# eric612/Mobilenet-YOLO-Pytorch

Hardware: AMD Instinct MI355X
Metric: images/sec MobileNetV2-YOLO 352x352 fwd+bwd @ bs256 (higher is better)
Workload: dtype f32; 1 GPU; MobileNetV2-YOLO 352x352 bs=256/GPU fwd+loss+bwd fp32 (BASELINE configs[1]); global_batch=256, parallelism=dp1

## Files before the change

### include/mnyolo.h

```cpp
#ifndef MNYOLO_H
#define MNYOLO_H

#include <stddef.h>
#include <stdint.h>

#ifdef __cplusplus
extern "C" {
#endif
#pragma GCC visibility push(default)

#define MNY_OK 0
#define MNY_EINVAL (-1)
#define MNY_EHIP (-2)
#define MNY_EUNSUPPORTED (-3)

#define MNY_ACT_NONE 0
#define MNY_ACT_RELU6 1
#define MNY_ACT_LEAKY 2
#define MNY_ACT_RELU 3
#define MNY_ACT_HSWISH 4
#define MNY_ACT_HSIGMOID 5

int mny_version(void);
const char* mny_last_error(void);
// ... 469 lines not shown
                     const float* w_exp, const float* e_scale, const float* e_shift, const float* e_mean, const float* e_invstd,
                     const float* e_gamma, const float* w_dw, const float* addend, float* dx, float* dw_exp, float* dgamma_e, float* dbeta_e,
                     float* dw_dw, float* dw_ws, float* ws, float* in_red, int N, int H, int W, int K, int C, int stride, void* stream);

int mny_stemdw_supported(int N, int H, int W, int Cout, int s_act, int d_act);
int mny_stemdw_bwd_parts(int N, int H, int W, int Cout);
size_t mny_stemdw_bwd_ws_floats(int N, int H, int W, int Cout);
int mny_stemdw_bwd(const float* gd, const float* d, const float* d_scale, const float* d_shift, int d_act, const float* d_coef,
                   const float* s, const float* s_scale, const float* s_shift, const float* s_mean, const float* s_invstd,
                   const float* s_gamma, int s_act, const float* x_nchw, const float* w_stem, const float* w_dw,
                   float* dw_stem, float* dgamma_s, float* dbeta_s, float* dw_dw, float* dw_ws, float* ws,
                   int N, int H, int W, int Cout, void* stream);

int mny_pj_bwd_supported(int64_t M, int Ki, int No, int d_act);
int mny_pj_bwd_parts(int64_t M, int Ki, int No);
int mny_pj_bwd(const float* g, const float* y, const float* coef, const float* d, const float* d_scale, const float* d_shift,
               const float* d_mean, const float* d_invstd, int d_act, const float* w, float* gd, float* dw, float* dw_ws, float* red,
               int64_t M, int Ki, int No, void* stream);
int mny_pj_bwd_supported_bf16(int64_t M, int Ki, int No, int d_act);
int mny_pj_bwd_parts_bf16(int64_t M, int Ki, int No);
int mny_pj_bwd_bf16(const void* g, const void* y, const float* coef, const void* d, const float* d_scale, const float* d_shift,
                    const float* d_mean, const float* d_invstd, int d_act, const float* w, void* gd, float* dw, float* dw_ws, float* red,
                    int64_t M, int Ki, int No, void* stream);

typedef struct mny_gate_cut_job {
    const float* w1;
    const float* w2;
    void* wq;
    int32_t C, R;
} mny_gate_cut_job;
int mny_gate_supported(int64_t M, int C, int R);
int mny_gate_parts(int64_t M);
int mny_gate_bwd_parts(int64_t M);
int mny_gate_bwd_red3_supported(int C, int R);
size_t mny_gate_wq_bytes(int C, int R);
int mny_gate_cut_batch_bf16(const mny_gate_cut_job* jobs, int njobs, void* stream);
int mny_gate_stats1_bf16(const void* y3, const float* s3, const float* b3, const void* wq, float* stats, int64_t M, int C, int R,
                         void* stream);
int mny_gate_stats2_bf16(const void* y3, const float* s3, const float* b3, const void* wq, const float* sc1, const float* sh1,
                         float* stats, int64_t M, int C, int R, void* stream);
int mny_gate_fwd_bf16(const void* y3, const float* s3, const float* b3, const void* wq, const float* sc1, const float* sh1,
                      const float* sc2, const float* sh2, const void* add_x, const float* add_scale, const float* add_shift,
                      int add_act, void* out, int64_t M, int C, int R, void* stream);
int mny_gate_bwd1_bf16(const void* y3, const float* s3, const float* b3, const void* dout, const void* wq, const float* sc1,
                       const float* sh1, const float* sc2, const float* sh2, const float* mean2, const float* invstd2, float* red2,
                       int64_t M, int C, int R, void* stream);
// ... 23 lines not shown
```

### mobilenet-yolo-pytorch_amd/_lib.py

```python
import ctypes
import os
from ctypes import c_char_p, c_double, c_float, c_int, c_int32, c_int64, c_size_t, c_void_p

from . import switches

HERE = os.path.dirname(os.path.abspath(__file__))
LIB_PATH = switches.get("MNY_LIB") or os.path.join(HERE, "libmnyolo.so")

ACT_NONE, ACT_RELU6, ACT_LEAKY, ACT_RELU, ACT_HSWISH, ACT_HSIGMOID = 0, 1, 2, 3, 4, 5
ROUTE_TILE_V1, ROUTE_DMA_F32, ROUTE_DMA_X6, ROUTE_THIN, ROUTE_WIDE, ROUTE_WGRAD_STREAM, ROUTE_WAVE16 = 0, 1, 2, 3, 4, 5, 6


class MnyError(RuntimeError):
    pass


class YoloHead(ctypes.Structure):
    _fields_ = [("N", c_int), ("g", c_int), ("A", c_int), ("C", c_int), ("n_anchors_all", c_int),
                ("ignore_thresh", c_float), ("iou_thresh", c_float), ("iou_weighting", c_float)]


P = c_void_p
_SIGS = {
    "mny_version": (c_int, []),
# ... 13 lines not shown
    "mny_dw_wgrad_parts": (c_int, [c_int] * 6),
    "mny_dw_bnbwd_supported": (c_int, [c_int, c_int]),
    "mny_dw_bnbwd_parts": (c_int, [c_int] * 4),
    "mny_dw_bnbwd_parts_k": (c_int, [c_int] * 6),
    "mny_dw_bnbwd": (c_int, [P, P, P, P, c_int, P, P, P, P, c_int, P, P, P, P, P, c_int, c_int, c_int, c_int, c_int, c_int, P]),
    "mny_dw_bnbwd_s2_parts": (c_int, [c_int] * 4),
    "mny_dw_bnbwd_s2": (c_int, [P, P, P, P, c_int, P, P, P, P, c_int, P, P, P, P, P, c_int, c_int, c_int, c_int, P]),
    "mny_dw_bnbwd_red": (c_int, [P, P, P, P, c_int, P, P, P, P, c_int, P, P, P, P, P, P, P, P, c_int, c_int, c_int, c_int, c_int, c_int, P]),
    "mny_exdw_supported": (c_int, [c_int] * 6),
    "mny_exdw_stat_parts": (c_int, [c_int64, c_int, c_int]),
    "mny_exdw_stats": (c_int, [P, P, P, c_int, P, P, c_int64, c_int, c_int, P]),
    "mny_exdw_fwd_parts": (c_int, [c_int] * 6),
    "mny_exdw_fwd": (c_int, [P, P, P, c_int, P, P, P, P, P, P, c_int, c_int, c_int, c_int, c_int, c_int, P]),
    "mny_exdw_bwd_parts": (c_int, [c_int] * 6),
    "mny_exdw_bwd_ws_floats": (c_size_t, [c_int] * 6),
    "mny_exdw_bwd": (c_int, [P, P, P, P, c_int, P, P, P, P, c_int, P, P, P, P, P, P, P, P, P, P, P, P, P, P, P,
                             c_int, c_int, c_int, c_int, c_int, c_int, P]),
    "mny_exdw_bwd_red_parts": (c_int, [c_int] * 6),
    "mny_exdw_bwd_red": (c_int, [P, P, P, P, c_int, P, P, P, P, c_int, P, P, P, P, P, P, P, P, P, P, P, P, P, P, P, P, P, P,
                                 c_int, c_int, c_int, c_int, c_int, c_int, P]),
    "mny_pj_bwd_supported": (c_int, [c_int64, c_int, c_int, c_int]),
    "mny_pj_bwd_parts": (c_int, [c_int64, c_int, c_int]),
    "mny_pj_bwd": (c_int, [P, P, P, P, P, P, P, P, c_int, P, P, P, P, P, c_int64, c_int, c_int, P]),
    "mny_stemdw_supported": (c_int, [c_int] * 6),
    "mny_stemdw_bwd_parts": (c_int, [c_int] * 4),
    "mny_stemdw_bwd_ws_floats": (c_size_t, [c_int] * 4),
    "mny_stemdw_bwd": (c_int, [P, P, P, P, c_int, P, P, P, P, P, P, P, c_int, P, P, P, P, P, P, P, P, P, c_int, c_int, c_int, c_int, P]),
    "mny_adamw_step": (c_int, [P, c_int, c_double, c_double, c_double, c_double, c_double, c_int64, P]),
    "mny_sgd_step": (c_int, [P, c_int, c_double, c_double, c_double, c_double, c_int, c_int, P]),
    "mny_ema_update": (c_int, [P, c_int, c_double, P]),
    "mny_swap_chunks": (c_int, [P, c_int, P]),
    "mny_grad_clip_parts": (c_int, [c_int64]),
    "mny_grad_clip": (c_int, [P, c_int, c_int, c_double, P, P, P]),
    "mny_pw_fwd": (c_int, [P, P, P, c_int, P, P, P, P, P, c_int64, c_int, c_int, P]),
    "mny_pw_stat_parts": (c_int, [c_int64, c_int, c_int]),
    "mny_pw_wgrad": (c_int, [P, P, P, c_int, P, P, P, P, c_int64, c_int, c_int, P]),
    "mny_pw_wgrad_ws_floats": (c_size_t, [c_int64, c_int, c_int]),
    "mny_pw_bnbwd_supported": (c_int, [c_int64, c_int, c_int]),
    "mny_pw_bnbwd_ws_floats": (c_size_t, [c_int64, c_int, c_int]),
    "mny_pw_bnbwd": (c_int, [P, P, P, P, c_int, P, P, P, P, P, P, c_int, P, P, P, P, P, P, P, c_int64, c_int, c_int, P]),
    "mny_pw_dgrad_bnred_supported": (c_int, [c_int64, c_int, c_int, c_int]),
    "mny_pw_dgrad_bnred_parts": (c_int, [c_int64, c_int, c_int]),
    "mny_pw_dgrad_bnred": (c_int, [P, P, P, P, P, P, c_int, P, P, P, c_int64, c_int, c_int, P]),
    "mny_pw_dgrad_bnred_add_supported": (c_int, [c_int64, c_int, c_int, c_int]),
    "mny_pw_dgrad_bnred_add": (c_int, [P, P, P, P, P, P, P, c_int, P, P, P, c_int64, c_int, c_int, P]),
    "mny_pw_route": (c_int, [c_int, c_int, c_int64, c_int, c_int]),
# ... 139 lines not shown
```

### mobilenet-yolo-pytorch_amd/csrc/common.h

```cpp
#pragma once
#include <hip/hip_runtime.h>
#include <stdint.h>
#include <stdio.h>
#include <stdlib.h>
#include <type_traits>

#include "../../include/mnyolo.h"

namespace mny {

void set_error(const char* fmt, ...);
int check_launch(const char* what);
bool allow_lds(const void* kernel, size_t bytes);

#define MNY_REQUIRE(cond, ...)                 \
    do {                                       \
        if (!(cond)) {                         \
            mny::set_error(__VA_ARGS__);       \
            return MNY_EINVAL;                 \
        }                                      \
    } while (0)

constexpr int kWave = 64;
constexpr int kMaxParts = 1024;
// ... 116 lines not shown
    if constexpr (B < E) {
        f(std::integral_constant<int, B>{});
        static_for<B + 1, E>(f);
    }
}
#define MNY_LGKM_WAIT(first) asm volatile("s_waitcnt lgkmcnt(0)" : "+v"(first))
#define MNY_LGKM_DEP(x) asm volatile("" : "+v"(x))

template <int N>
__device__ __forceinline__ void wait_vmcnt() { asm volatile("s_waitcnt vmcnt(%0)" ::"n"(N) : "memory"); }

#define MNY_SWITCHES(X)                                                                                                              \
    X(GEMM_V1, "MNY_GEMM_V1", kFlag, 0, 1, "pointwise forward / data gradients on the first-generation tile kernels")                \
    X(WGRAD_V1, "MNY_WGRAD_V1", kFlag, 0, 1, "pointwise weight gradients on the first-generation tile kernel")                       \
    X(WGRAD_NO_XCD, "MNY_WGRAD_NO_XCD", kFlag, 0, 1, "weight-gradient workgroups in plain order, not grouped per XCD")               \
    X(X6, "MNY_X6", kInt, -1, 1, "six-product bf16 GEMM: 0 = never (fp32 MFMA), 1 = wherever supported, -1 = per-shape rule")        \
    X(NO_W6, "MNY_NO_W6", kFlag, 0, 1, "no pre-cut weight operand for the six-product GEMM")                                         \
    X(NO_WIDE, "MNY_NO_WIDE", kFlag, 0, 1, "no barrier-free short-reduction kernel (pwwide.hip)")                                    \
    X(NO_WGS, "MNY_NO_WGS", kFlag, 0, 1, "no stream weight-gradient kernel (pwwgs.hip)")                                             \
    X(NO_THIN, "MNY_NO_THIN", kFlag, 0, 1, "no vector-ALU kernel for K = 8..32 (pwthin.hip)")                                        \
    X(NO_PWT, "MNY_NO_PWT", kFlag, 0, 1, "no wave-per-16-pixels thin pointwise kernel (gate.hip)")                                   \
    X(NO_PWE, "MNY_NO_PWE", kFlag, 0, 1, "no wave form of the thin expand unit backward (gate.hip)")                                 \
    X(NO_PJBWD, "MNY_NO_PJBWD", kFlag, 0, 1, "no fused projection backward (pjbwd.hip, gate.hip)")                                   \
    X(NO_LR, "MNY_NO_LR", kFlag, 0, 1, "no low-rank BatchNorm backward of the wide expand units (lrbwd.hip)")                        \
    X(NO_EXDW, "MNY_NO_EXDW", kFlag, 0, 1, "no fused expand + depthwise unit: the materialised path")                                \
    X(EXDW_STATS, "MNY_EXDW_STATS", kWord, 0, 0, "gram (default) | direct: how mny_exdw_stats forms its sums")                       \
    X(NO_STEMDW, "MNY_NO_STEMDW", kFlag, 0, 1, "no fused stem + depthwise backward (stemdw.hip)")                                    \
    X(STEM_WGRAD_VALU, "MNY_STEM_WGRAD_VALU", kFlag, 0, 1, "stem weight gradient on the vector ALU, not the matrix cores")           \
    X(DW_V1, "MNY_DW_V1", kFlag, 0, 1, "3x3 depthwise forward on the first-generation sliding-window kernel")                        \
    X(NO_DWT5, "MNY_NO_DWT5", kFlag, 0, 1, "no tile form of the 5x5 depthwise unit backward")                                        \
    X(DWT3, "MNY_DWT3", kInt, -1, 1, "tile form of the 3x3 depthwise unit backward: 0 / 1, -1 = per-shape rule")                     \
    X(DWTF, "MNY_DWTF", kInt, -1, 1, "tile form of the depthwise forward: 0 / 1, -1 = per-shape rule")                               \
    X(NMS_SMALL, "MNY_NMS_SMALL", kFlag, 0, 0, "NMS buckets of any size through the one-workgroup path")
enum SwitchType { kFlag, kInt, kWord };
enum Switch {
#define X(id, name, type, def, latch, doc) SW_##id,
    MNY_SWITCHES(X)
#undef X
    SW_COUNT
};
int sw(Switch id);

struct CgLayout {
    int cg_total;
    int chunks;
    int cgb;
// ... 79 lines not shown
```

### mobilenet-yolo-pytorch_amd/csrc/pwwide.hip

```cpp
#include <mutex>
#include <vector>

#include "common.h"
#include "x6.h"

namespace mny {

struct WideArgs {
    const float* A; const float* in_scale; const float* in_shift; int in_act;
    const float* W;
    float* C; float* stats;
    int64_t M; int K, N;
    int gx, n_blocks; int64_t ntiles;
    const float* rY; const float* r_scale; const float* r_shift; const float* r_mean; const float* r_invstd; int r_act;
    const float* addend;
    const float* bias;
};

template <int KS, int TNB, int XF, int MODE>
__global__ __launch_bounds__(256) __attribute__((amdgpu_waves_per_eu(2, 2))) void pw_wide_kernel(WideArgs p) {
    constexpr int BN = 32 * TNB;
    constexpr bool TWO_ACC = false;
    extern __shared__ __attribute__((aligned(16))) float smem[];
    float* sB = smem;
    float* sScale = sB + TNB * KS * 3 * 256;
    float* sShift = sScale + KS * 16;
    const int tid = threadIdx.x, lane = tid & 63;
    const int wave = __builtin_amdgcn_readfirstlane(tid >> 6);
    const int lrow = lane & 31, khalf = lane >> 5;
    const int bid = blockIdx.x, xcd = bid & 7, local = bid >> 3;
    const int y = local % p.n_blocks, x = (local / p.n_blocks) * 8 + xcd;
    if (x >= p.gx) return;
    const int n0 = y * BN;
    const int K = p.K, N = p.N;

    for (int c = tid; c < TNB * KS * 64; c += 256) {
        const int sidx = c >> 6, l = c & 63, j = l & 31, h = l >> 5;
        const int u = sidx / KS, s = sidx - u * KS;
        const int n = n0 + u * 32 + j;
        const int k0 = s * 16 + 4 * h, k1 = k0 + 8;
        const float* src = p.W + (int64_t)(n < N ? n : 0) * K;
        const float4 v0 = (n < N && k0 < K) ? ld4(src + k0) : f4zero();
        const float4 v1 = (n < N && k1 < K) ? ld4(src + k1) : f4zero();
        bf16x8_t hh, mm, ll;
        x6_split(v4f_t{v0.x, v0.y, v0.z, v0.w}, v4f_t{v1.x, v1.y, v1.z, v1.w}, hh, mm, ll);
        float* dst = sB + (sidx * 3) * 256 + l * 4;
        *reinterpret_cast<v4f_t*>(dst) = __builtin_bit_cast(v4f_t, hh);
        *reinterpret_cast<v4f_t*>(dst + 256) = __builtin_bit_cast(v4f_t, mm);
        *reinterpret_cast<v4f_t*>(dst + 512) = __builtin_bit_cast(v4f_t, ll);
    }
    if ((XF != 0 && MODE < 2) || MODE == 4) {
        const bool has = p.in_scale != nullptr;
        for (int k = tid; k < KS * 16; k += 256) {
            sScale[k] = k < K ? (has ? p.in_scale[k] : 1.f) : 0.f;
            sShift[k] = (k < K && has) ? p.in_shift[k] : 0.f;
        }
    }
    __syncthreads();

    const float slope = act_slope(p.in_act), hi = act_hi(p.in_act);
    const int quad = lrow >> 2, jq = lane & 3;
    const float rslope = act_slope(p.r_act), rhi = act_hi(p.r_act);
    const bool rhsig = p.r_act == MNY_ACT_HSIGMOID;
    float s1[TNB], s2[TNB];
#pragma unroll
    for (int u = 0; u < TNB; ++u) { s1[u] = 0.f; s2[u] = 0.f; }

    const float* bl = sB + lane * 4;
    const float* scl = sScale + 4 * khalf;
    const float* shl = sShift + 4 * khalf;
    const int64_t nslots = (int64_t)p.gx * 4;
    const unsigned rowb = (unsigned)N * 4u;
    float4 g[2 * KS];
    float ry[MODE >= 2 ? 16 : 1], ra[MODE >= 3 ? 16 : 1];
    auto load_g = [&](int64_t tile, int s) {
        const int64_t r = tile * 32 + lrow;
        const float* row = p.A + (r < p.M ? r : p.M - 1) * K;
        int k0 = 16 * s + 4 * khalf, k1 = k0 + 8;
        if (s == KS - 1) { k0 = k0 < K ? k0 : 0; k1 = k1 < K ? k1 : 0; }
        g[2 * s] = ld4(row + k0); g[2 * s + 1] = ld4(row + k1);
    };
    auto load_r = [&](int64_t tile, int u) {
        const int col = n0 + u * 32 + lrow, cc = col < N ? col : 0;
        unsigned voff = (unsigned)(4 * khalf) * rowb + (unsigned)cc * 4u;
        asm volatile("" : "+v"(voff));
        const float* ub = p.rY + tile * 32 * N;
#pragma unroll
        for (int r = 0; r < 16; ++r) ry[r] = ld1(at_bytes(ub + (int64_t)(8 * (r >> 2) + (r & 3)) * N, voff));
        if constexpr (MODE >= 3) {
            const float* ua = p.addend + tile * 32 * N;
#pragma unroll
            for (int r = 0; r < 16; ++r) ra[r] = ld1(at_bytes(ua + (int64_t)(8 * (r >> 2) + (r & 3)) * N, voff));
        }
    };

    auto do_tile = [&](const int64_t tile, const int64_t next) {
        const int64_t wrow = tile * 32;
        bf16x8_t ah[KS], am[KS], al[KS];
#pragma unroll
        for (int s = 0; s < KS; ++s) {
            const float4 a0 = g[2 * s], a1 = g[2 * s + 1];
            float z[8] = {a0.x, a0.y, a0.z, a0.w, a1.x, a1.y, a1.z, a1.w};
            if ((XF != 0 && MODE < 2) || MODE == 4) {
                v4f_t c0 = *reinterpret_cast<const v4f_t*>(scl + 16 * s), c1 = *reinterpret_cast<const v4f_t*>(scl + 16 * s + 8);
                v4f_t h0 = *reinterpret_cast<const v4f_t*>(shl + 16 * s), h1 = *reinterpret_cast<const v4f_t*>(shl + 16 * s + 8);
                asm volatile("s_waitcnt lgkmcnt(0)" : "+v"(c0), "+v"(c1), "+v"(h0), "+v"(h1));
                const float sv[8] = {c0.x, c0.y, c0.z, c0.w, c1.x, c1.y, c1.z, c1.w}, hv[8] = {h0.x, h0.y, h0.z, h0.w, h1.x, h1.y, h1.z, h1.w};
#pragma unroll
                for (int e = 0; e < 8; ++e) {
                    const float t = fmaf(z[e], sv[e], hv[e]);
                    z[e] = MODE == 4 ? t : (XF == 1 ? fminf(fmaxf(t, slope * t), hi) : t * fminf(fmaxf(t + 3.f, 0.f), 6.f) * (1.f / 6.f));
                }
            }
            x6_split(v4f_t{z[0], z[1], z[2], z[3]}, v4f_t{z[4], z[5], z[6], z[7]}, ah[s], am[s], al[s]);
            asm volatile("" : "+v"(ah[s]), "+v"(am[s]), "+v"(al[s]) :: "memory");
            load_g(next, s);
            __builtin_amdgcn_sched_barrier(0);
        }
        float* cbase = p.C + wrow * N;
#pragma unroll
        for (int u = 0; u < TNB; ++u) {
            float4 rc = f4zero();
            float cbias = 0.f;
            if (MODE >= 2) {
                const int colx = n0 + u * 32 + lrow;
                rc = make_float4(p.r_scale[colx], p.r_shift[colx], p.r_mean[colx], p.r_invstd[colx]);
                if (MODE == 4) cbias = p.bias[colx];
            }
            f32x16 acc, acc1;
#pragma unroll
            for (int r = 0; r < 16; ++r) { acc[r] = 0.f; acc1[r] = 0.f; }
#pragma unroll
            for (int s = 0; s < KS; ++s) {
                const float* bsrc = bl + ((u * KS + s) * 3) * 256;
                const bf16x8_t bh = __builtin_bit_cast(bf16x8_t, *reinterpret_cast<const v4f_t*>(bsrc));
                const bf16x8_t bm = __builtin_bit_cast(bf16x8_t, *reinterpret_cast<const v4f_t*>(bsrc + 256));
                const bf16x8_t bl_ = __builtin_bit_cast(bf16x8_t, *reinterpret_cast<const v4f_t*>(bsrc + 512));
                f32x16& a = (TWO_ACC && (s & 1)) ? acc1 : acc;
                a = __builtin_amdgcn_mfma_f32_32x32x16_bf16(al[s], bh, a, 0, 0, 0);
                a = __builtin_amdgcn_mfma_f32_32x32x16_bf16(ah[s], bl_, a, 0, 0, 0);
                a = __builtin_amdgcn_mfma_f32_32x32x16_bf16(am[s], bm, a, 0, 0, 0);
                a = __builtin_amdgcn_mfma_f32_32x32x16_bf16(am[s], bh, a, 0, 0, 0);
                a = __builtin_amdgcn_mfma_f32_32x32x16_bf16(ah[s], bm, a, 0, 0, 0);
                a = __builtin_amdgcn_mfma_f32_32x32x16_bf16(ah[s], bh, a, 0, 0, 0);
            }
            if (TWO_ACC) {
#pragma unroll
                for (int r = 0; r < 16; ++r) acc[r] += acc1[r];
            }
            if (MODE >= 2) {
#pragma unroll
                for (int r = 0; r < 16; ++r) {
                    const float zz = fmaf(ry[r], rc.x, rc.y);
                    float dact;
                    if (XF == 0) dact = (zz > 0.f ? 1.f : rslope) * (zz < rhi ? 1.f : 0.f);
                    else {
                        const float dsw = zz <= -3.f ? 0.f : (zz >= 3.f ? 1.f : fmaf(zz, 1.f / 3.f, 0.5f));
                        const float dsg = (zz > -3.f && zz < 3.f) ? (1.f / 6.f) : 0.f;
                        dact = rhsig ? dsg : dsw;
                    }
                    if (MODE >= 3) acc[r] += ra[r];
                    if (MODE == 4) acc[r] += cbias;
                    const float dz = acc[r] * dact;
                    s1[u] += dz; s2[u] = fmaf(dz, (ry[r] - rc.z) * rc.w, s2[u]);
                }
                asm volatile("" : "+v"(acc) :: "memory");
                if (u + 1 < TNB) load_r(tile, u + 1); else load_r(next, 0);
                __builtin_amdgcn_sched_barrier(0);
            } else if (MODE == 1) {
                v2f a1 = v2f{0.f, 0.f}, a2 = v2f{0.f, 0.f};
#pragma unroll
                for (int r = 0; r < 16; r += 2) {
                    const v2f q = v2f{acc[r], acc[r + 1]};
                    a1 += q;
                    a2 = __builtin_elementwise_fma(q, q, a2);
                }
                s1[u] += a1.x + a1.y; s2[u] += a2.x + a2.y;
            }
            unsigned off0 = (unsigned)(4 * khalf + jq) * rowb + (unsigned)(n0 + u * 32 + quad * 4) * 4u;
            asm volatile("" : "+v"(off0));
#pragma unroll
            for (int gq = 0; gq < 4; ++gq) {
                float r0 = acc[gq * 4 + 0], r1 = acc[gq * 4 + 1], r2 = acc[gq * 4 + 2], r3 = acc[gq * 4 + 3];
                {
                    const bool odd = lane & 1;
                    const float xa = odd ? r0 : r1, xb = odd ? r2 : r3;
                    const float ya = __builtin_bit_cast(float, __builtin_amdgcn_mov_dpp(__builtin_bit_cast(int, xa), 0xB1, 0xF, 0xF, true));
                    const float yb = __builtin_bit_cast(float, __builtin_amdgcn_mov_dpp(__builtin_bit_cast(int, xb), 0xB1, 0xF, 0xF, true));
                    if (odd) { r0 = ya; r2 = yb; } else { r1 = ya; r3 = yb; }
                }
                {
                    const bool hi2 = lane & 2;
                    const float xa = hi2 ? r0 : r2, xb = hi2 ? r1 : r3;
                    const float ya = __builtin_bit_cast(float, __builtin_amdgcn_mov_dpp(__builtin_bit_cast(int, xa), 0x4E, 0xF, 0xF, true));
                    const float yb = __builtin_bit_cast(float, __builtin_amdgcn_mov_dpp(__builtin_bit_cast(int, xb), 0x4E, 0xF, 0xF, true));
                    if (hi2) { r0 = ya; r1 = yb; } else { r2 = ya; r3 = yb; }
                }
                st4(at_bytes(cbase + (int64_t)(8 * gq) * N, off0), make_float4(r0, r1, r2, r3));
            }
            __builtin_amdgcn_sched_barrier(0);
        }
    };

    int64_t tile = (int64_t)x * 4 + wave;
    if (tile < p.ntiles) {
#pragma unroll
        for (int s = 0; s < KS; ++s) load_g(tile, s);
        if (MODE >= 2) load_r(tile, 0);
    }
    if (tile < p.ntiles) {
        do_tile(tile, tile + nslots < p.ntiles ? tile + nslots : tile);
        tile += nslots;
        for (; tile < p.ntiles; tile += nslots) do_tile(tile, tile + nslots < p.ntiles ? tile + nslots : tile);
    }

    if (MODE != 0) {
        __syncthreads();
        float* red = smem;
#pragma unroll
        for (int u = 0; u < TNB; ++u) {
            const float a = s1[u] + __shfl_xor(s1[u], 32);
            const float b = s2[u] + __shfl_xor(s2[u], 32);
            if (khalf == 0) {
                red[(wave * BN + u * 32 + lrow) * 2 + 0] = a;
                red[(wave * BN + u * 32 + lrow) * 2 + 1] = b;
            }
        }
        __syncthreads();
        if (tid < BN) {
            float a = 0.f, b = 0.f;
#pragma unroll
            for (int w = 0; w < 4; ++w) { a += red[(w * BN + tid) * 2]; b += red[(w * BN + tid) * 2 + 1]; }
            p.stats[(int64_t)x * 2 * N + n0 + tid] = a;
            p.stats[(int64_t)x * 2 * N + N + n0 + tid] = b;
        }
    }
}

struct WidePlan { int KS, TNB, n_blocks, gx, grid; int64_t ntiles; size_t lds; };

static bool wide_on() {
    return !sw(SW_NO_WIDE) && !sw(SW_GEMM_V1);
}

static int wide_tnb(int , int N, bool red) {
    const int cap = red ? 3 : 4;
    if (N % 96 == 0 && cap >= 3) return 3;
    if (N % 128 == 0 && cap >= 4) return 4;
    return N % 64 == 0 ? 2 : 0;
}

bool pw_wide_ok(int64_t M, int K, int N, bool red) {
    return wide_on() && M >= 8192 && K >= 52 && K <= 96 && (K & 3) == 0 && N >= 64 && wide_tnb(K, N, red) != 0 && N >= K;
}

static WidePlan wide_plan(int64_t M, int K, int N, bool red) {
    WidePlan pl;
    pl.KS = (K + 15) / 16;
// ... 64 lines not shown

int pw_wide_launch(const float* A, const float* in_scale, const float* in_shift, int in_act, const float* W, float* C, float* stats,
                   int64_t M, int K, int N, const float* rY, const float* r_scale, const float* r_shift, const float* r_mean,
                   const float* r_invstd, int r_act, const float* addend, hipStream_t st) {
    MNY_REQUIRE(pw_wide_ok(M, K, N, rY != nullptr) && (M & 31) == 0, "pw_wide: unsupported problem M=%lld K=%d N=%d (whole 32-row tiles: callers send the last M %% 32 rows elsewhere)", (long long)M, K, N);
    const WidePlan pl = wide_plan(M, K, N, rY != nullptr);
    MNY_REQUIRE(pl.KS >= 4 && pl.KS <= 6 && pl.TNB >= 2 && pl.TNB <= 4, "pw_wide: no kernel for K=%d, column block %d", K, 32 * pl.TNB);
    const bool xf = in_scale != nullptr || in_act != MNY_ACT_NONE;
    const int mode = rY ? (addend ? 3 : 2) : (stats ? 1 : 0);
    const int XF = rY ? (r_act >= MNY_ACT_HSWISH ? 2 : 0) : (!xf ? 0 : (in_act == MNY_ACT_HSWISH ? 2 : 1));
    MNY_REQUIRE(!(rY && xf), "pw_wide: the reduction form takes its A operand as is");
    MNY_REQUIRE(!rY || r_act < MNY_ACT_HSWISH, "pw_wide: the reduction form knows the clamp family only (mny_pw_dgrad_bnred_supported)");
    MNY_REQUIRE(rY || !addend, "pw_wide: a plain addend is not supported (callers route it to the LDS-DMA kernel)");
    MNY_REQUIRE(in_act != MNY_ACT_HSIGMOID, "pw_wide: h-sigmoid input transform is not supported");
    WideArgs a{A, in_scale, in_shift, in_act, W, C, stats, M, K, N, pl.gx, pl.n_blocks, pl.ntiles, rY, r_scale, r_shift, r_mean, r_invstd, r_act, addend, nullptr};
    const WideKernel k = wide_pick(pl.KS, pl.TNB, XF, mode);
    if (!allow_lds((const void*)k, 80 * 1024)) {
        set_error("pw_wide: hipFuncSetAttribute failed"); return MNY_EHIP;
    }
    hipLaunchKernelGGL(k, dim3(pl.grid), dim3(256), pl.lds, st, a);
    return check_launch("pw_wide_kernel");
}

}
```

### mobilenet-yolo-pytorch_amd/engine.py

```python
import ctypes
import itertools
import os
import re
import warnings

import numpy as np
import torch

from . import _lib, frontier, switches
from ._lib import ACT_NONE, MnyError, YoloHead

_FWD_TICK = itertools.count()

BN_EPS = 1e-5
BN_MOMENTUM = 0.1
_vp = ctypes.c_void_p


def _ptr(t):
    return _vp(t.data_ptr()) if t is not None else None


class CallList:

# ... 863 lines not shown
        return _lib.query("mny_lr_supported", self._rows(pn.out), pi.C, pn.out.C) == 1

    def _bwd_emitter(self, nd):
        o = nd.out
        if o.id in self.gates:
            return self._bwd_gate
        if nd.op == "dw" and o.id in self.exdw_dw:
            return self._bwd_exdw
        if nd.op in ("add", "mul", "partadd"):
            return {"add": self._bwd_add, "mul": self._bwd_mul, "partadd": self._bwd_partadd}[nd.op]
        if nd.op == "pw" and self._takes_own_sums(nd):
            return self._bwd_thin_expand
        if nd.op == "pw" and o.id in self.lr_units:
            return self._bwd_lr_expand
        if nd.op == "dw" and o.act != _lib.ACT_HSIGMOID and nd.ins[0].act != _lib.ACT_HSIGMOID:
            if _lib.query("mny_dw_bnbwd_supported", nd.k, nd.stride) == 1:
                return self._bwd_dw_s1
            if nd.k == 3 and nd.stride == 2:
                return self._bwd_dw_s2
            if nd.k == 5 and nd.stride == 2 and not self.sw_no_dwfuse5s2 and o.C % 2 == 0:
                return self._bwd_dw_s2k5
        if self._project_ok(nd):
            return self._bwd_project
        return self._bwd_generic

    def _bwd_gate(self, nd, G):
        bwd, P, gv, eb, gs = self.bwd, self._P, self._gv, self.eb, self._gs
        gate = self.gates[nd.out.id]
        t, se0, se3 = gate["t"], gate["se0"], gate["se3"]
        if gate["add"] is not None:
            self._contribute_alias(gate["add"].ins[1], G)
        u1, u2, u3 = self.units[se0.out.id], self.units[se3.out.id], self.units[t.id]
        tv = self._view(t)
        M, C, R = self._rows(nd.out), t.C, se0.out.C
        wq = gate["wq"]
        gparts = _lib.query("mny_gate_bwd_parts", M)
        coef2, coef1 = torch.empty(3 * C, **self._f32), torch.empty(3 * R, **self._f32)
        gate["coef"] = (coef2, coef1)
        bwd.add("mny_gate_bwd1_bf16", tv[0], tv[1], tv[2], G, wq, u1.scale, u1.shift, u2.scale, u2.shift, u2.mean, u2.invstd, self.red_ws, M, C, R, self.stream,
                meta=dict(flops=4 * M * C * R, bytes=eb * 2 * M * C, shape="gate bwd1 M%d C%d R%d" % (M, C, R)))
        bwd.add(self.fin_name, self.red_ws, gparts, M, P[se3.bn + ".weight"], u2.mean, u2.invstd, gv(se3.bn + ".weight"), gv(se3.bn + ".bias"), coef2, C, self.stream)
        ws2 = self._defer_job(gparts * C * R, gv(se3.conv + ".weight"), gparts, C * R)
        bwd.add("mny_gate_bwd2_bf16", tv[0], tv[1], tv[2], G, wq, u1.scale, u1.shift, u1.mean, u1.invstd, u2.scale, u2.shift, coef2, self.red_ws, ws2,
                M, C, R, self.stream, meta=dict(flops=8 * M * C * R, bytes=eb * 2 * M * C, shape="gate bwd2 M%d C%d R%d" % (M, C, R)))
        bwd.add(self.fin_name, self.red_ws, gparts, M, P[se0.bn + ".weight"], u1.mean, u1.invstd, gv(se0.bn + ".weight"), gv(se0.bn + ".bias"), coef1, R, self.stream)
        ws1 = self._defer_job(gparts * C * R, gv(se0.conv + ".weight"), gparts, C * R)
# ... 202 lines not shown
        else:
            self._contribute_kernel(i, lambda out, addend: self.bwd.add(
                self.K("mny_dw_bnbwd_s2"), *head, wt, addend, out, dwv_k, ws_k, N, ish[1], ish[2], C, self.stream, meta=meta))

    def _bwd_dw_s2k5(self, nd, G):
        N = self.N
        o, u, i = nd.out, self.units[nd.out.id], nd.ins[0]
        M, C = u.M, o.C
        ish = self._shape(i)
        xv = self._view(i)
        self._bn_sums(nd, G)
        wt = self._P[nd.conv + ".weight"]
        dparts = _lib.query("mny_dw_bnbwd_s2k5_parts", N, ish[1], ish[2], C)
        dwv_k, ws_k = self._wgrad_dest(nd, dparts, C * 25, self.ws)
        pmean, pinvstd, rbuf = None, None, None
        if self._sole_producer(i, xv, ("pw", "stem"), no_acts=(_lib.ACT_HSIGMOID,)):
            pmean, pinvstd = self.units[i.id].mean, self.units[i.id].invstd
            rbuf = self._new_fused_red(i, dparts)
        self._contribute_kernel(i, lambda out, addend: self.bwd.add(
            self.K("mny_dw_bnbwd_s2k5"), G, u.Y, u.scale, u.shift, o.act, self.coef_ws, xv[0], xv[1], xv[2], xv[3], pmean, pinvstd, wt, addend, out, dwv_k, ws_k, rbuf,
            N, ish[1], ish[2], C, self.stream,
            meta=dict(flops=4 * M * C * 25, bytes=self.eb * (2 * M * C + 2 * N * ish[1] * ish[2] * C), shape="C%d H%d s2 k5%s" % (C, ish[1], " +red" if rbuf is not None else ""))))

    def _project_ok(self, nd):
        o = nd.out
        if not (nd.op == "pw" and not self.frozen and o.act == ACT_NONE and not nd.bias and self._single(nd) and o.id not in self.head_cp):
            return False
        i = nd.ins[0]
        return (self._sole_producer(i, self._view(i), ("dw", "pw"), need_single=True)
                and _lib.query(self.K("mny_pj_bwd_supported"), self.units[o.id].M, i.C, o.C, i.act) == 1)

    def _bwd_project(self, nd, G):
        o, u, i = nd.out, self.units[nd.out.id], nd.ins[0]
        M, Ki, No = u.M, i.C, o.C
        self._bn_sums(nd, G)
        pu = self.units[i.id]
        rparts = _lib.query(self.K("mny_pj_bwd_parts"), M, Ki, No)
        rbuf = self._new_fused_red(i, rparts)
        dwv_k, ws_k = self._wgrad_dest(nd, rparts, No * Ki, None)
        self._contribute_kernel(i, lambda out, addend: self.bwd.add(
            self.K("mny_pj_bwd"), G, u.Y, self.coef_ws, pu.Y, pu.scale, pu.shift, pu.mean, pu.invstd, i.act, self._P[nd.conv + ".weight"], out, dwv_k, ws_k, rbuf,
            M, Ki, No, self.stream,
            meta=dict(flops=4 * M * Ki * No, bytes=self.eb * (2 * M * No + 2 * M * Ki), shape="project M%d K%d N%d" % (M, Ki, No))))

    def _bwd_generic(self, nd, G):
        bwd, o = self.bwd, nd.out
        if nd.op == "pwb":
            return self._bwd_pw_grads(nd, G)
        u = self.units[o.id]
        dY = G if not self._gs[o.id].shared else self._alloc_grad(o)
        self._bn_sums(nd, G)
        if nd.op == "stem" and _lib.query("mny_stem_bnwgrad_supported", o.C) == 1:
            sdw, sws = self._wgrad_dest(nd, lambda: _lib.query("mny_stem_wgrad_parts", self.N, self.H, self.W, o.C), o.C * 27, self.ws)
            bwd.add(self.K("mny_stem_bnwgrad"), self.x_ptr, G, u.Y, u.scale, u.shift, o.act, self.coef_ws, sdw, sws,
                    self.N, self.H, self.W, o.C, self.stream)
            return
        bwd.add(self.K("mny_bn_bwd_apply"), G, u.Y, u.scale, u.shift, o.act, self.coef_ws, dY, u.M, o.C, self.stream,
                meta=dict(flops=0, bytes=3 * self.eb * u.M * o.C, shape="M%d C%d" % (u.M, o.C)))
        if nd.op == "stem":
            if self.side_on:
                bwd.add_py(self._fork_side, "fork")
            bwd.add(self.K("mny_stem_wgrad"), self.x_ptr, dY, self._gv(nd.conv + ".weight"), self.ws_side, self.N, self.H, self.W, o.C, self.stream_side)
        elif nd.op == "dw":
            self._bwd_dw_grads(nd, dY)
# ... 274 lines not shown
```

### mobilenet-yolo-pytorch_amd/switches.py

```python
import os
import warnings

FLAG, INT, WORD, TEXT = "flag", "int", "word", "text"

TABLE = (
    ("MNY_LIB", TEXT, None, "loader", "path of another libmnyolo.so build to load (A/B on one machine)"),
    ("MNY_HIPGRAPH", FLAG, 0, "plan", "replay training plans through captured hipGraphs"),
    ("MNY_SIDE_STREAM", INT, None, "plan", "weight gradients on a side stream: 0 / 1, unset = up to 48 M input pixels"),
    ("MNY_NO_GATE", FLAG, 0, "plan", "per-pixel gates as separate convs, BatchNorms and a multiply, not fused units"),
    ("MNY_EXDW_K", TEXT, "16,24", "plan", "input widths whose expand + depthwise pairs run as one unit"),
    ("MNY_NO_LR", FLAG, 0, "plan lib", "no low-rank BatchNorm backward of the wide expand units (lrbwd.hip)"),
    ("MNY_NO_LR_S2", FLAG, 0, "plan", "no low-rank BatchNorm backward behind the stride-2 depthwise units"),
    ("MNY_NO_DWFUSE5S2", FLAG, 0, "plan", "5x5 stride-2 depthwise units on the generic backward kernels"),
    ("MNY_GEMM_V1", FLAG, 0, "lib", "pointwise forward / data gradients on the first-generation tile kernels"),
    ("MNY_WGRAD_V1", FLAG, 0, "lib", "pointwise weight gradients on the first-generation tile kernel"),
    ("MNY_WGRAD_NO_XCD", FLAG, 0, "lib", "weight-gradient workgroups in plain order, not grouped per XCD"),
    ("MNY_X6", INT, -1, "lib", "six-product bf16 GEMM: 0 = never (fp32 MFMA), 1 = wherever supported, -1 = per-shape rule"),
    ("MNY_NO_W6", FLAG, 0, "lib", "no pre-cut weight operand for the six-product GEMM"),
    ("MNY_NO_WIDE", FLAG, 0, "lib", "no barrier-free short-reduction kernel (pwwide.hip)"),
    ("MNY_NO_WGS", FLAG, 0, "lib", "no stream weight-gradient kernel (pwwgs.hip)"),
    ("MNY_NO_THIN", FLAG, 0, "lib", "no vector-ALU kernel for K = 8..32 (pwthin.hip)"),
    ("MNY_NO_PWT", FLAG, 0, "lib", "no wave-per-16-pixels thin pointwise kernel (gate.hip)"),
    ("MNY_NO_PWE", FLAG, 0, "lib", "no wave form of the thin expand unit backward (gate.hip)"),
    ("MNY_NO_PJBWD", FLAG, 0, "lib", "no fused projection backward (pjbwd.hip, gate.hip)"),
    ("MNY_NO_EXDW", FLAG, 0, "lib", "no fused expand + depthwise unit: the materialised path"),
    ("MNY_EXDW_STATS", WORD, 0, "lib", "gram (default) | direct: how mny_exdw_stats forms its sums"),
    ("MNY_NO_STEMDW", FLAG, 0, "lib", "no fused stem + depthwise backward (stemdw.hip)"),
    ("MNY_STEM_WGRAD_VALU", FLAG, 0, "lib", "stem weight gradient on the vector ALU, not the matrix cores"),
    ("MNY_DW_V1", FLAG, 0, "lib", "3x3 depthwise forward on the first-generation sliding-window kernel"),
    ("MNY_NO_DWT5", FLAG, 0, "lib", "no tile form of the 5x5 depthwise unit backward"),
    ("MNY_DWT3", INT, -1, "lib", "tile form of the 3x3 depthwise unit backward: 0 / 1, -1 = per-shape rule"),
    ("MNY_DWTF", INT, -1, "lib", "tile form of the depthwise forward: 0 / 1, -1 = per-shape rule"),
    ("MNY_NMS_SMALL", FLAG, 0, "lib", "NMS buckets of any size through the one-workgroup path"),
    ("MNY_FORCE_DP", FLAG, 0, "bench", "bench.py: run the RCCL data-parallel path even with one rank"),
    ("MNY_LAUNCHER_PARENT_CLEAN", FLAG, 0, "bench", "bench.py: set by its launcher for the rank processes it starts"),
    ("MNY_PRINT_MARKS", FLAG, 0, "bench", "bench.py: print the backward call list's marks"),
)
_ROWS = {row[0]: row for row in TABLE}


def get(name):
    _, kind, default, _, _ = _ROWS[name]
    raw = os.environ.get(name)
    if kind == FLAG:
        return raw not in (None, "", "0")
    if raw in (None, ""):
        return default
# ... 9 lines not shown
```

Before: 7375 images/s.

## Fuse projection weight gradient into wide pointwise data-gradient kernel

Adds a weight-gradient variant of the wide barrier-free pointwise kernel for project units with 64 outputs. It computes the data gradient with the preceding BatchNorm backward and, in the same pass, accumulates the weight gradient with six-product bf16 MFMAs over the recomputed activation and the incoming gradient. It then folds per-wave partials through LDS and writes per-block partial rows that are reduced afterwards. This removes a separate weight-gradient GEMM pass that re-reads the same activations. In exchange it adds register and LDS pressure, strided column loads of the gradient, and an extra BN-apply launch before the kernel.

```diff
diff --git a/include/mnyolo.h b/include/mnyolo.h
--- a/include/mnyolo.h
+++ b/include/mnyolo.h
@@ -515,6 +515,10 @@
 int mny_pj_bwd_bf16(const void* g, const void* y, const float* coef, const void* d, const float* d_scale, const float* d_shift,
                     const float* d_mean, const float* d_invstd, int d_act, const float* w, void* gd, float* dw, float* dw_ws, float* red,
                     int64_t M, int Ki, int No, void* stream);
+int mny_pjw_bwd_supported(int64_t M, int Ki, int No, int d_act);
+int mny_pjw_bwd_parts(int64_t M, int Ki, int No);
+int mny_pjw_bwd(const float* dy, const float* d, const float* d_scale, const float* d_shift, const float* d_mean, const float* d_invstd,
+                int d_act, const float* w, float* gd, float* dw, float* dw_ws, float* red, int64_t M, int Ki, int No, void* stream);
 
 typedef struct mny_gate_cut_job {
     const float* w1;
diff --git a/mobilenet-yolo-pytorch_amd/_lib.py b/mobilenet-yolo-pytorch_amd/_lib.py
--- a/mobilenet-yolo-pytorch_amd/_lib.py
+++ b/mobilenet-yolo-pytorch_amd/_lib.py
@@ -59,6 +59,9 @@
     "mny_pj_bwd_supported": (c_int, [c_int64, c_int, c_int, c_int]),
     "mny_pj_bwd_parts": (c_int, [c_int64, c_int, c_int]),
     "mny_pj_bwd": (c_int, [P, P, P, P, P, P, P, P, c_int, P, P, P, P, P, c_int64, c_int, c_int, P]),
+    "mny_pjw_bwd_supported": (c_int, [c_int64, c_int, c_int, c_int]),
+    "mny_pjw_bwd_parts": (c_int, [c_int64, c_int, c_int]),
+    "mny_pjw_bwd": (c_int, [P, P, P, P, P, P, c_int, P, P, P, P, P, c_int64, c_int, c_int, P]),
     "mny_stemdw_supported": (c_int, [c_int] * 6),
     "mny_stemdw_bwd_parts": (c_int, [c_int] * 4),
     "mny_stemdw_bwd_ws_floats": (c_size_t, [c_int] * 4),
diff --git a/mobilenet-yolo-pytorch_amd/csrc/common.h b/mobilenet-yolo-pytorch_amd/csrc/common.h
--- a/mobilenet-yolo-pytorch_amd/csrc/common.h
+++ b/mobilenet-yolo-pytorch_amd/csrc/common.h
@@ -162,6 +162,7 @@
     X(NO_PWT, "MNY_NO_PWT", kFlag, 0, 1, "no wave-per-16-pixels thin pointwise kernel (gate.hip)")                                   \
     X(NO_PWE, "MNY_NO_PWE", kFlag, 0, 1, "no wave form of the thin expand unit backward (gate.hip)")                                 \
     X(NO_PJBWD, "MNY_NO_PJBWD", kFlag, 0, 1, "no fused projection backward (pjbwd.hip, gate.hip)")                                   \
+    X(NO_PJW, "MNY_NO_PJW", kFlag, 0, 1, "no weight gradient inside the wide project-unit data gradient (pwwide.hip)")               \
     X(NO_LR, "MNY_NO_LR", kFlag, 0, 1, "no low-rank BatchNorm backward of the wide expand units (lrbwd.hip)")                        \
     X(NO_EXDW, "MNY_NO_EXDW", kFlag, 0, 1, "no fused expand + depthwise unit: the materialised path")                                \
     X(EXDW_STATS, "MNY_EXDW_STATS", kWord, 0, 0, "gram (default) | direct: how mny_exdw_stats forms its sums")                       \
diff --git a/mobilenet-yolo-pytorch_amd/csrc/pwwide.hip b/mobilenet-yolo-pytorch_amd/csrc/pwwide.hip
--- a/mobilenet-yolo-pytorch_amd/csrc/pwwide.hip
+++ b/mobilenet-yolo-pytorch_amd/csrc/pwwide.hip
@@ -15,11 +15,14 @@
     const float* rY; const float* r_scale; const float* r_shift; const float* r_mean; const float* r_invstd; int r_act;
     const float* addend;
     const float* bias;
+    float* dwp;
 };
 
-template <int KS, int TNB, int XF, int MODE>
+template <int KS, int TNB, int XF, int MODE, int WG = 0>
 __global__ __launch_bounds__(256) __attribute__((amdgpu_waves_per_eu(2, 2))) void pw_wide_kernel(WideArgs p) {
+    static_assert(WG == 0 || (MODE == 2 && XF == 0 && KS == 2 * (WG > 0 ? WG : KS / 2)), "the weight-gradient form: MODE 2, clamp family, K = 32 WG");
     constexpr int BN = 32 * TNB;
+    constexpr int NI = WG > 0 ? WG : 0;
     constexpr bool TWO_ACC = false;
     extern __shared__ __attribute__((aligned(16))) float smem[];
     float* sB = smem;
@@ -40,8 +43,15 @@
         const int n = n0 + u * 32 + j;
         const int k0 = s * 16 + 4 * h, k1 = k0 + 8;
         const float* src = p.W + (int64_t)(n < N ? n : 0) * K;
-        const float4 v0 = (n < N && k0 < K) ? ld4(src + k0) : f4zero();
-        const float4 v1 = (n < N && k1 < K) ? ld4(src + k1) : f4zero();
+        float4 v0, v1;
+        if constexpr (WG != 0) {
+            const float* col = p.W + n;
+            v0 = make_float4(col[(int64_t)k0 * N], col[(int64_t)(k0 + 1) * N], col[(int64_t)(k0 + 2) * N], col[(int64_t)(k0 + 3) * N]);
+            v1 = make_float4(col[(int64_t)k1 * N], col[(int64_t)(k1 + 1) * N], col[(int64_t)(k1 + 2) * N], col[(int64_t)(k1 + 3) * N]);
+        } else {
+            v0 = (n < N && k0 < K) ? ld4(src + k0) : f4zero();
+            v1 = (n < N && k1 < K) ? ld4(src + k1) : f4zero();
+        }
         bf16x8_t hh, mm, ll;
         x6_split(v4f_t{v0.x, v0.y, v0.z, v0.w}, v4f_t{v1.x, v1.y, v1.z, v1.w}, hh, mm, ll);
         float* dst = sB + (sidx * 3) * 256 + l * 4;
@@ -69,10 +79,30 @@
     const float* bl = sB + lane * 4;
     const float* scl = sScale + 4 * khalf;
     const float* shl = sShift + 4 * khalf;
+    float* sAl = sShift + KS * 16 + (NI > 0 ? wave * (KS * 2 * 256) + lane * 4 : 0);
     const int64_t nslots = (int64_t)p.gx * 4;
     const unsigned rowb = (unsigned)N * 4u;
     float4 g[2 * KS];
     float ry[MODE >= 2 ? 16 : 1], ra[MODE >= 3 ? 16 : 1];
+    f32x16 dwa[NI > 0 ? NI : 1][NI > 0 ? TNB : 1];
+    float cr[2][NI > 0 ? 8 : 1];
+    if constexpr (NI > 0) {
+#pragma unroll
+        for (int i = 0; i < NI; ++i)
+#pragma unroll
+            for (int u = 0; u < TNB; ++u)
+#pragma unroll
+                for (int r = 0; r < 16; ++r) dwa[i][u][r] = 0.f;
+    }
+    auto load_c = [&](int64_t tile, int t) {
+        const int ks = t / (NI > 0 ? NI : 1), i = t - ks * NI;
+        constexpr int KC = 16 * KS;
+        unsigned voff = ((unsigned)(4 * khalf) * (unsigned)KC + (unsigned)lrow) * 4u;
+        asm volatile("" : "+v"(voff));
+        const float* ub = p.A + tile * (32 * KC);
+#pragma unroll
+        for (int e = 0; e < 8; ++e) cr[t & 1][e] = ld1(at_bytes(ub + (16 * ks + 8 * (e >> 2) + (e & 3)) * KC + 32 * i, voff));
+    };
     auto load_g = [&](int64_t tile, int s) {
         const int64_t r = tile * 32 + lrow;
         const float* row = p.A + (r < p.M ? r : p.M - 1) * K;
@@ -114,6 +144,10 @@
             }
             x6_split(v4f_t{z[0], z[1], z[2], z[3]}, v4f_t{z[4], z[5], z[6], z[7]}, ah[s], am[s], al[s]);
             asm volatile("" : "+v"(ah[s]), "+v"(am[s]), "+v"(al[s]) :: "memory");
+            if constexpr (NI > 0) {
+                *reinterpret_cast<v4f_t*>(sAl + (2 * s) * 256) = __builtin_bit_cast(v4f_t, ah[s]);
+                *reinterpret_cast<v4f_t*>(sAl + (2 * s + 1) * 256) = __builtin_bit_cast(v4f_t, am[s]);
+            }
             load_g(next, s);
             __builtin_amdgcn_sched_barrier(0);
         }
@@ -130,6 +164,26 @@
             f32x16 acc, acc1;
 #pragma unroll
             for (int r = 0; r < 16; ++r) { acc[r] = 0.f; acc1[r] = 0.f; }
+            if constexpr (NI > 0) {
+#pragma unroll
+                for (int s = 0; s < KS; ++s) {
+                    const float* bsrc = bl + ((u * KS + s) * 3) * 256;
+                    const bf16x8_t bh = __builtin_bit_cast(bf16x8_t, *reinterpret_cast<const v4f_t*>(bsrc));
+                    const bf16x8_t bm = __builtin_bit_cast(bf16x8_t, *reinterpret_cast<const v4f_t*>(bsrc + 256));
+                    const bf16x8_t bl_ = __builtin_bit_cast(bf16x8_t, *reinterpret_cast<const v4f_t*>(bsrc + 512));
+                    const bf16x8_t xh = __builtin_bit_cast(bf16x8_t, *reinterpret_cast<const v4f_t*>(sAl + (2 * s) * 256));
+                    const bf16x8_t xm = __builtin_bit_cast(bf16x8_t, *reinterpret_cast<const v4f_t*>(sAl + (2 * s + 1) * 256));
+                    acc = __builtin_amdgcn_mfma_f32_32x32x16_bf16(al[s], bh, acc, 0, 0, 0);
+                    acc = __builtin_amdgcn_mfma_f32_32x32x16_bf16(xh, bl_, acc, 0, 0, 0);
+                    acc = __builtin_amdgcn_mfma_f32_32x32x16_bf16(xm, bm, acc, 0, 0, 0);
+                    acc = __builtin_amdgcn_mfma_f32_32x32x16_bf16(xm, bh, acc, 0, 0, 0);
+                    acc = __builtin_amdgcn_mfma_f32_32x32x16_bf16(xh, bm, acc, 0, 0, 0);
+                    acc = __builtin_amdgcn_mfma_f32_32x32x16_bf16(xh, bh, acc, 0, 0, 0);
+                    __builtin_amdgcn_sched_barrier(0);
+                }
+                load_c(tile, 0);
+                load_c(tile, 1);
+            } else
 #pragma unroll
             for (int s = 0; s < KS; ++s) {
                 const float* bsrc = bl + ((u * KS + s) * 3) * 256;
@@ -163,10 +217,13 @@
                     if (MODE == 4) acc[r] += cbias;
                     const float dz = acc[r] * dact;
                     s1[u] += dz; s2[u] = fmaf(dz, (ry[r] - rc.z) * rc.w, s2[u]);
-                }
-                asm volatile("" : "+v"(acc) :: "memory");
-                if (u + 1 < TNB) load_r(tile, u + 1); else load_r(next, 0);
-                __builtin_amdgcn_sched_barrier(0);
+                    if constexpr (NI > 0) ry[r] = fminf(fmaxf(zz, rslope * zz), rhi);
+                }
+                if constexpr (NI == 0) {
+                    asm volatile("" : "+v"(acc) :: "memory");
+                    if (u + 1 < TNB) load_r(tile, u + 1); else load_r(next, 0);
+                    __builtin_amdgcn_sched_barrier(0);
+                }
             } else if (MODE == 1) {
                 v2f a1 = v2f{0.f, 0.f}, a2 = v2f{0.f, 0.f};
 #pragma unroll
@@ -199,6 +256,33 @@
                 st4(at_bytes(cbase + (int64_t)(8 * gq) * N, off0), make_float4(r0, r1, r2, r3));
             }
             __builtin_amdgcn_sched_barrier(0);
+            if constexpr (NI > 0) {
+#pragma unroll
+                for (int ks = 0; ks < 2; ++ks) {
+                    bf16x8_t ph, pm, pl;
+                    x6_split(v4f_t{ry[8 * ks], ry[8 * ks + 1], ry[8 * ks + 2], ry[8 * ks + 3]}, v4f_t{ry[8 * ks + 4], ry[8 * ks + 5], ry[8 * ks + 6], ry[8 * ks + 7]}, ph, pm, pl);
+                    asm volatile("" : "+v"(ph), "+v"(pm), "+v"(pl) :: "memory");
+#pragma unroll
+                    for (int i = 0; i < NI; ++i) {
+                        bf16x8_t ch, cm, cl;
+                        const float* c = cr[(ks * NI + i) & 1];
+                        x6_split(v4f_t{c[0], c[1], c[2], c[3]}, v4f_t{c[4], c[5], c[6], c[7]}, ch, cm, cl);
+                        asm volatile("" : "+v"(ch), "+v"(cm), "+v"(cl) :: "memory");
+                        if (ks * NI + i + 2 < 2 * NI) load_c(tile, ks * NI + i + 2);
+                        else if (ks * NI + i + 1 < 2 * NI) {}
+                        else if (u + 1 < TNB) load_r(tile, u + 1);
+                        else load_r(next, 0);
+                        f32x16& a = dwa[i][u];
+                        a = __builtin_amdgcn_mfma_f32_32x32x16_bf16(cl, ph, a, 0, 0, 0);
+                        a = __builtin_amdgcn_mfma_f32_32x32x16_bf16(ch, pl, a, 0, 0, 0);
+                        a = __builtin_amdgcn_mfma_f32_32x32x16_bf16(cm, pm, a, 0, 0, 0);
+                        a = __builtin_amdgcn_mfma_f32_32x32x16_bf16(cm, ph, a, 0, 0, 0);
+                        a = __builtin_amdgcn_mfma_f32_32x32x16_bf16(ch, pm, a, 0, 0, 0);
+                        a = __builtin_amdgcn_mfma_f32_32x32x16_bf16(ch, ph, a, 0, 0, 0);
+                        __builtin_amdgcn_sched_barrier(0);
+                    }
+                }
+            }
         }
     };
 
@@ -234,6 +318,29 @@
             p.stats[(int64_t)x * 2 * N + n0 + tid] = a;
             p.stats[(int64_t)x * 2 * N + N + n0 + tid] = b;
         }
+    }
+    if constexpr (NI > 0) {
+        float* fold = smem;
+        float* dst = p.dwp + (int64_t)x * K * N;
+#pragma unroll
+        for (int i = 0; i < NI; ++i)
+#pragma unroll
+            for (int u = 0; u < TNB; ++u) {
+                __syncthreads();
+                if (wave > 0) {
+#pragma unroll
+                    for (int r = 0; r < 16; ++r) fold[((wave - 1) * 16 + r) * 64 + lane] = dwa[i][u][r];
+                }
+                __syncthreads();
+                if (wave == 0) {
+#pragma unroll
+                    for (int r = 0; r < 16; ++r) {
+                        const float v = ((dwa[i][u][r] + fold[(0 * 16 + r) * 64 + lane]) + fold[(1 * 16 + r) * 64 + lane]) + fold[(2 * 16 + r) * 64 + lane];
+                        const int k = 32 * i + (r & 3) + 8 * (r >> 2) + 4 * khalf;
+                        dst[(int64_t)k * N + n0 + u * 32 + lrow] = v;
+                    }
+                }
+            }
     }
 }
 
@@ -344,4 +451,42 @@
     return check_launch("pw_wide_kernel");
 }
 
-}
+static bool pjw_shape_ok(int64_t M, int Ki, int No) {
+    return M >= 32 && (M & 31) == 0 && No == 64 && Ki >= No && wide_tnb(No, Ki, true) != 0;
+}
+template <int WG>
+static WideKernel pjw_pick(int TNB) {
+    if (TNB == 3) return pw_wide_kernel<4, 3, 0, 2, WG>;
+    return TNB == 2 ? pw_wide_kernel<4, 2, 0, 2, WG> : nullptr;
+}
+
+}
+
+using namespace mny;
+
+extern "C" int mny_pjw_bwd_supported(int64_t M, int Ki, int No, int d_act) {
+    return (wide_on() && !sw(SW_NO_PJW) && pjw_shape_ok(M, Ki, No) && d_act >= MNY_ACT_NONE && d_act < MNY_ACT_HSWISH) ? 1 : 0;
+}
+
+extern "C" int mny_pjw_bwd_parts(int64_t M, int Ki, int No) { return pjw_shape_ok(M, Ki, No) ? wide_plan(M, No, Ki, true).gx : MNY_EINVAL; }
+
+extern "C" int mny_pjw_bwd(const float* dy, const float* d, const float* d_scale, const float* d_shift, const float* d_mean, const float* d_invstd,
+                           int d_act, const float* w, float* gd, float* dw, float* dw_ws, float* red, int64_t M, int Ki, int No, void* stream) {
+    MNY_REQUIRE(dy && d && d_scale && d_shift && d_mean && d_invstd && w && gd && red, "pjw_bwd: null pointer");
+    MNY_REQUIRE(!dw || dw_ws, "pjw_bwd: a weight gradient needs its partial rows (dw_ws)");
+    MNY_REQUIRE(pjw_shape_ok(M, Ki, No) && d_act >= MNY_ACT_NONE && d_act < MNY_ACT_HSWISH, "pjw_bwd: M=%lld Ki=%d No=%d act %d not supported (mny_pjw_bwd_supported)",
+                (long long)M, Ki, No, d_act);
+    WidePlan pl = wide_plan(M, No, Ki, true);
+    if (dw_ws) pl.lds += (size_t)4 * pl.KS * 2 * 256 * sizeof(float);
+    WideArgs a{dy, nullptr, nullptr, MNY_ACT_NONE, w, gd, red, M, No, Ki, pl.gx, pl.n_blocks, pl.ntiles, d, d_scale, d_shift, d_mean, d_invstd, d_act, nullptr, nullptr, dw_ws};
+    const WideKernel k = dw_ws ? pjw_pick<2>(pl.TNB) : pjw_pick<-1>(pl.TNB);
+    MNY_REQUIRE(k != nullptr, "pjw_bwd: no kernel for a column block of %d", 32 * pl.TNB);
+    if (!allow_lds((const void*)k, 80 * 1024)) {
+        set_error("pjw_bwd: hipFuncSetAttribute failed"); return MNY_EHIP;
+    }
+    hipStream_t st = (hipStream_t)stream;
+    hipLaunchKernelGGL(k, dim3(pl.grid), dim3(256), pl.lds, st, a);
+    const int rc = check_launch("pw_wide_kernel<pjw>");
+    if (rc || !dw) return rc;
+    return launch_reduce_parts(dw_ws, pl.gx, No * Ki, dw, st);
+}
diff --git a/mobilenet-yolo-pytorch_amd/engine.py b/mobilenet-yolo-pytorch_amd/engine.py
--- a/mobilenet-yolo-pytorch_amd/engine.py
+++ b/mobilenet-yolo-pytorch_amd/engine.py
@@ -909,6 +909,8 @@
                 return self._bwd_dw_s2k5
         if self._project_ok(nd):
             return self._bwd_project
+        if self._project_ok(nd, "mny_pjw_bwd_supported"):
+            return self._bwd_project_wide
         return self._bwd_generic
 
     def _bwd_gate(self, nd, G):
@@ -1157,13 +1159,15 @@
             N, ish[1], ish[2], C, self.stream,
             meta=dict(flops=4 * M * C * 25, bytes=self.eb * (2 * M * C + 2 * N * ish[1] * ish[2] * C), shape="C%d H%d s2 k5%s" % (C, ish[1], " +red" if rbuf is not None else ""))))
 
-    def _project_ok(self, nd):
+    def _project_ok(self, nd, supported=None):
         o = nd.out
         if not (nd.op == "pw" and not self.frozen and o.act == ACT_NONE and not nd.bias and self._single(nd) and o.id not in self.head_cp):
             return False
+        if supported is not None and (self.bf16 or not self.frontier.needs_grad(nd.ins[0])):
+            return False
         i = nd.ins[0]
         return (self._sole_producer(i, self._view(i), ("dw", "pw"), need_single=True)
-                and _lib.query(self.K("mny_pj_bwd_supported"), self.units[o.id].M, i.C, o.C, i.act) == 1)
+                and _lib.query(supported or self.K("mny_pj_bwd_supported"), self.units[o.id].M, i.C, o.C, i.act) == 1)
 
     def _bwd_project(self, nd, G):
         o, u, i = nd.out, self.units[nd.out.id], nd.ins[0]
@@ -1175,6 +1179,23 @@
         dwv_k, ws_k = self._wgrad_dest(nd, rparts, No * Ki, None)
         self._contribute_kernel(i, lambda out, addend: self.bwd.add(
             self.K("mny_pj_bwd"), G, u.Y, self.coef_ws, pu.Y, pu.scale, pu.shift, pu.mean, pu.invstd, i.act, self._P[nd.conv + ".weight"], out, dwv_k, ws_k, rbuf,
+            M, Ki, No, self.stream,
+            meta=dict(flops=4 * M * Ki * No, bytes=self.eb * (2 * M * No + 2 * M * Ki), shape="project M%d K%d N%d" % (M, Ki, No))))
+
+    def _bwd_project_wide(self, nd, G):
+        o, u, i = nd.out, self.units[nd.out.id], nd.ins[0]
+        M, Ki, No = u.M, i.C, o.C
+        dY = G if not self._gs[o.id].shared else self._alloc_grad(o)
+        self._bn_sums(nd, G)
+        self.bwd.add(self.K("mny_bn_bwd_apply"), G, u.Y, u.scale, u.shift, o.act, self.coef_ws, dY, M, No, self.stream,
+                     meta=dict(flops=0, bytes=3 * self.eb * M * No, shape="M%d C%d" % (M, No)))
+        pu = self.units[i.id]
+        rparts = _lib.query("mny_pjw_bwd_parts", M, Ki, No)
+        rbuf = self._new_fused_red(i, rparts)
+        dwv_k, ws_k = self._wgrad_dest(nd, rparts, No * Ki, self.ws)
+        assert dwv_k is None
+        self._contribute_kernel(i, lambda out, addend: self.bwd.add(
+            "mny_pjw_bwd", dY, pu.Y, pu.scale, pu.shift, pu.mean, pu.invstd, i.act, self._P[nd.conv + ".weight"], out, dwv_k, ws_k, rbuf,
             M, Ki, No, self.stream,
             meta=dict(flops=4 * M * Ki * No, bytes=self.eb * (2 * M * No + 2 * M * Ki), shape="project M%d K%d N%d" % (M, Ki, No))))
 
diff --git a/mobilenet-yolo-pytorch_amd/switches.py b/mobilenet-yolo-pytorch_amd/switches.py
--- a/mobilenet-yolo-pytorch_amd/switches.py
+++ b/mobilenet-yolo-pytorch_amd/switches.py
@@ -23,6 +23,7 @@
     ("MNY_NO_PWT", FLAG, 0, "lib", "no wave-per-16-pixels thin pointwise kernel (gate.hip)"),
     ("MNY_NO_PWE", FLAG, 0, "lib", "no wave form of the thin expand unit backward (gate.hip)"),
     ("MNY_NO_PJBWD", FLAG, 0, "lib", "no fused projection backward (pjbwd.hip, gate.hip)"),
+    ("MNY_NO_PJW", FLAG, 0, "lib", "no weight gradient inside the wide project-unit data gradient (pwwide.hip)"),
     ("MNY_NO_EXDW", FLAG, 0, "lib", "no fused expand + depthwise unit: the materialised path"),
     ("MNY_EXDW_STATS", WORD, 0, "lib", "gram (default) | direct: how mny_exdw_stats forms its sums"),
     ("MNY_NO_STEMDW", FLAG, 0, "lib", "no fused stem + depthwise backward (stemdw.hip)"),
```

Result: no change. 7373 images/s (-0.0%).
